# kdexd/probnmn-clevr

Hardware: AMD Instinct MI355X
Metric: CLEVR questions/sec (joint_training step) (higher is better)
Workload: dtype f32; 1 GPU; joint_training_ours.yml (NMN + seq2seq + REINFORCE), global batch 1024 = 1024 questions per GPU x 1 (BASELINE configs[3]), 14x14x1024 features, half of the batch with program supervision, fwd+bwd+[all-reduce]+clamp+Adam; global_batch=1024, per_gpu_batch=1024, parallelism=dp1

## Files before the change

include/probnmn_hip.h:

```cpp
#ifndef PROBNMN_HIP_H
#define PROBNMN_HIP_H

#include <stdint.h>

#ifdef __cplusplus
extern "C" {
#endif

#define PNMN_EINVAL (-1)
#define PNMN_ESHAPE (-2)

#define PNMN_CHANNELS 128

typedef struct pnmn_conv_item {
    const float* in;
    const float* in2;
    const float* mask;
    const float* gate;
    const float* weight;
    const float* bias;
    float*       out;
    int32_t      dilation;
    int32_t      flags;
    const float* mb_feats;
// ... 111 lines not shown
int pnmn_gather_features(const float* store, const int64_t* indices, float* dst, int n, int64_t n_store,
                         int C, int HW, void* stream);
int pnmn_copy_rows_h2d(const void* store, const int64_t* indices, void* dst, int n, int64_t n_store,
                       int64_t row_bytes, void* stream);

int pnmn_maxpool2_flatten_fwd(const float* in, float* out, int n, int H, int W, int C, void* stream);
int pnmn_maxpool2_flatten_bwd(const float* in, const float* dout, float* din, int n, int H, int W,
                              int C, void* stream);

int pnmn_answer_loss(const float* logits, const int64_t* answers, const int32_t* valid,
                     int64_t* predictions, float* loss, float* dlogits, int n, int num_answers,
                     int unknown_index, float scale, void* stream);

typedef struct {
    const float* src;
    const float* src2;
    float* dst;
    int32_t n, k, ld, kind;
} pnmn_derive_job;

int pnmn_token_prep(const int64_t* tokens, int64_t token_row_stride, int B, int T, int pad, int bos, int eos,
                    int drop_first, int64_t* out, float* fmask, int* last, void* stream);
int pnmn_length_order(const int32_t* last, int B, int T, int32_t* order, int32_t* tile_steps, void* stream);
int pnmn_trim_predictions(const int64_t* raw, int B, int T, int end, int64_t* out, void* stream);
int pnmn_mask_last_fwd(const float* hs, const float* fmask, const int* last, int B, int T, int H, float* enc,
                       float* hlast, void* stream);
int pnmn_mask_last_bwd(const float* denc, const float* dhlast, const float* fmask, const int* last, int B, int T,
                       int H, float* dhs, void* stream);
int64_t pnmn_embedding_grad_workspace_bytes(int B, int T, int V);
int pnmn_embedding_grad(const float* dy, const int64_t* tokens, int64_t token_row_stride, int B, int T, int C,
                        int V, int shift, int start, int skip, int accumulate, float* dw, void* workspace, void* stream);
int pnmn_derive_params(const pnmn_derive_job* jobs, int n_jobs, int max_quads, void* stream);

int pnmn_token_table_fwd(const float* emb, const float* weight, int64_t weight_row_stride,
                         const float* bias, int V, int K, int N, float* table, void* stream);
int pnmn_token_table_bwd(const float* dtable, const float* emb, const float* weight,
                         int64_t weight_row_stride, int V, int K, int N, int padding_idx, float* demb,
                         float* dweight, int64_t dweight_row_stride , float* dbias,
                         float* dbias2 , void* stream);

#define PNMN_TOKEN_SEGS 4
typedef struct pnmn_token_seg {
    const int64_t* src;
    const int64_t* index;
    int64_t        row_stride;
    int32_t        rows;
// ... 287 lines not shown
#define PNMN_GEMM_A_TRANSPOSED 1
#define PNMN_GEMM_B_TRANSPOSED 2
#define PNMN_GEMM_ACCUMULATE   4
typedef struct pnmn_gemm_desc {
    const float* a;
    const float* b;
    float*       c;
    const float* bias;
    int64_t      lda, ldb, ldc;
    int32_t      M, N, K;
    int32_t      flags;
    int32_t      split_k;
    int32_t      shift_t;
    const float* shift_h0;
    int64_t      ld_h0;
    float*       workspace;
    float*       colsum;
    float*       colsum2;
} pnmn_gemm_desc;
int pnmn_gemm(const pnmn_gemm_desc* descs , int n, void* stream);
int pnmn_gemm_cus(const pnmn_gemm_desc* descs , int n, int max_workgroups, void* stream);
int64_t pnmn_gemm_workspace_bytes(int M, int N, int split_k);
int pnmn_gemm_split_k(int M, int N, int K, int cus);

int pnmn_colsum(const float* x, int64_t ld, int R, int C, float* out, float* out2, int accumulate, void* workspace, void* stream);
int64_t pnmn_colsum_workspace_bytes(int R, int C);

#define PNMN_ABI_VERSION 13
int pnmn_abi_version(void);

#ifdef __cplusplus
}
#endif
#endif
```

probnmn-clevr_amd/csrc/gemm.hip:

```cpp
#include <hip/hip_runtime.h>
#include <stdint.h>

#include <type_traits>

#include "../../include/probnmn_hip.h"
#include "global_ptr.h"
#include "lds_optin.h"

namespace {

typedef float f32x16 __attribute__((ext_vector_type(16)));
using pnmn::as_global;
using pnmn::gfloat;

constexpr int TM = 128, TN = 128, TK = 32;
constexpr int OP_FLOATS = TM * TK;
using lchar = __attribute__((address_space(3))) char;
using gchar = __attribute__((address_space(1))) char;

struct Batch {
    pnmn_gemm_desc d[PNMN_GEMM_MAX];
    int first[PNMN_GEMM_MAX + 1];
    int n;
};
// ... 100 lines not shown
            const int c = (lane & 7) ^ (lane >> 4);
            base = o + ((int64_t)(row0 + 32 * wave) * ld + k0) * 4;
            v0 = (uint32_t)((lane >> 3) * ld) * 4u + 16u * c, v1 = (uint32_t)((lane >> 3) * ld) * 4u + 16u * (c ^ 4);
            piece = 32 * ld, step = 4 * TK, off = (uint32_t)wave * 32u * 128u;
        } else {
            base = o + ((int64_t)(k0 + 8 * wave) * ld + row0) * 4;
            v0 = v1 = (uint32_t)((lane >> 5) * ld) * 4u + 16u * (lane & 31);
            piece = 8 * ld, step = 4 * (int64_t)TK * ld, off = (uint32_t)wave * 8u * 512u;
        }
    }
    __device__ __forceinline__ void issue(float* tile) {
        const uint32_t dst = __builtin_amdgcn_readfirstlane((uint32_t)(uintptr_t)((lchar*)tile)) + off;
#pragma unroll
        for (int j = 0; j < 4; ++j) {
            const uint64_t src = (uint64_t)(uintptr_t)(base + j * piece);
            asm volatile("s_mov_b32 m0, %2\n\ts_nop 0\n\tglobal_load_lds_dwordx4 %0, %1"
                         :
                         : "v"(KC && (j & 1) ? v1 : v0), "s"(src), "s"(dst + 1024u * j)
                         : "memory");
        }
        base += step;
    }
};

template <bool AKC, bool BKC>
__device__ __forceinline__ void contract(const pnmn_gemm_desc& d, int m0, int n0, int kbeg, int kend, float* lds, f32x16 (&acc)[2][2],
                                         bool want_cs, float (&cs)[2]) {
    const int tid = threadIdx.x, wave = tid >> 6, lane = tid & 63, i = lane & 31, h = lane >> 5;
    const int wm = wave >> 1, wn = wave & 1;
    const gfloat* A = as_global(d.a);
    const gfloat* Bm = as_global(d.b);
    const gfloat* h0 = as_global(d.shift_h0);
    const bool avec = (d.lda & 3) == 0 && ((uintptr_t)d.a & 15) == 0;
    const bool bvec = (d.ldb & 3) == 0 && ((uintptr_t)d.b & 15) == 0 && (d.shift_t == 0 || d.shift_h0 == nullptr ||
                                                                       ((d.ld_h0 & 3) == 0 && ((uintptr_t)d.shift_h0 & 15) == 0));
    float* la = lds;
    float* lb = lds + 2 * OP_FLOATS;
    const bool adir = avec && m0 + TM <= d.M, bdir = bvec && n0 + TN <= d.N && (BKC || d.shift_t == 0);
    const int kfull = kbeg + (kend - kbeg) / TK * TK;
    const float rcp_t = d.shift_t > 0 ? 1.f / (float)d.shift_t : 0.f;
    Direct<AKC> da;
    Direct<BKC> db;
    da.start(A, d.lda, m0, kbeg, tid);
    db.start(Bm, d.ldb, n0, kbeg, tid);
    auto loop = [&](auto ad_tag, auto bd_tag, int lo, int hi) {
        constexpr bool AD = decltype(ad_tag)::value, BD = decltype(bd_tag)::value;
// ... 5 lines not shown
                load_tile<AKC>(A, d.lda, m0, k0, d.M, kend, avec, tid, ra, 0, nullptr, 0);
            if constexpr (BD)
                db.issue(lb + st * OP_FLOATS);
            else if constexpr (AD && !BKC)
                load_tile_shift(Bm, d.ldb, n0, k0, tid, rb, d.shift_t, rcp_t, h0, d.ld_h0);
            else
                load_tile<BKC>(Bm, d.ldb, n0, k0, d.N, kend, bvec, tid, rb, BKC ? 0 : d.shift_t, h0, d.ld_h0);
        };
        auto commit = [&](int st) {
            if constexpr (!AD) store_tile<AKC>(la + st * OP_FLOATS, tid, ra);
            if constexpr (!BD) store_tile<BKC>(lb + st * OP_FLOATS, tid, rb);
        };
        if (lo >= hi) return;
        fetch(lo, 0);
        commit(0);
        asm volatile("s_waitcnt vmcnt(0)" ::: "memory");
        __syncthreads();
        int cur = 0;
        for (int k0 = lo; k0 < hi; k0 += TK) {
            const bool more = k0 + TK < hi;
            if (more) fetch(k0 + TK, cur ^ 1);
            const float* ca = la + cur * OP_FLOATS;
            const float* cb = lb + cur * OP_FLOATS;
#pragma unroll
            for (int q = 0; q < 4; ++q) {
                f32x4 a[2], b[2];
#pragma unroll
                for (int t = 0; t < 2; ++t) {
                    a[t] = frag<AKC>(ca, 64 * wm + 32 * t + i, q, h);
                    b[t] = frag<BKC>(cb, 64 * wn + 32 * t + i, q, h);
                }
                if (!AKC && want_cs) {
#pragma unroll
                    for (int t = 0; t < 2; ++t) cs[t] += (a[t][0] + a[t][1]) + (a[t][2] + a[t][3]);
                }
#pragma unroll
                for (int s = 0; s < 4; ++s)
#pragma unroll
                    for (int mt = 0; mt < 2; ++mt)
#pragma unroll
                        for (int nt = 0; nt < 2; ++nt)
                            acc[mt][nt] = __builtin_amdgcn_mfma_f32_32x32x2f32(a[mt][s], b[nt][s], acc[mt][nt], 0, 0, 0);
            }
            if (more) commit(cur ^ 1);
            asm volatile("s_waitcnt vmcnt(0)" ::: "memory");
            __syncthreads();
            cur ^= 1;
        }
    };
    using yes = std::true_type;
    using no = std::false_type;
    if (adir && bdir) {
        loop(yes{}, yes{}, kbeg, kfull);
        loop(no{}, no{}, kfull, kend);
    } else if (!BKC && adir && bvec && d.shift_t > 0 && n0 + TN <= d.N && kend <= (1 << 21)) {
        if constexpr (!BKC) {
            loop(yes{}, no{}, kbeg, kfull);
            loop(no{}, no{}, kfull, kend);
        }
    } else {
        loop(no{}, no{}, kbeg, kend);
    }
}

__global__ __launch_bounds__(256) __attribute__((amdgpu_waves_per_eu(2, 2))) void gemm_kernel(const Batch batch) {
    extern __shared__ __attribute__((aligned(16))) float lds[];
    for (int unit = blockIdx.x; unit < batch.first[batch.n]; unit += gridDim.x) {
    int pi = 0;
    while (pi + 1 < batch.n && unit >= batch.first[pi + 1]) ++pi;
    const pnmn_gemm_desc d = batch.d[pi];
    const int local = unit - batch.first[pi];
    const int tiles_n = (d.N + TN - 1) / TN, tiles_m = (d.M + TM - 1) / TM;
    const int split = d.split_k > 1 ? d.split_k : 1;
    const int chunk = local % split, tile = local / split;
    const int tm = tile / tiles_n, tn = tile % tiles_n;
    const int m0 = tm * TM, n0 = tn * TN;
    const int ktiles = (d.K + TK - 1) / TK;
    const int per = ktiles / split, extra = ktiles % split;
    const int kt0 = chunk * per + (chunk < extra ? chunk : extra);
    const int kt1 = kt0 + per + (chunk < extra ? 1 : 0);
    const int kbeg = kt0 * TK, kend = kt1 * TK < d.K ? kt1 * TK : d.K;

    f32x16 acc[2][2];
#pragma unroll
    for (int mt = 0; mt < 2; ++mt)
#pragma unroll
        for (int nt = 0; nt < 2; ++nt)
#pragma unroll
            for (int r = 0; r < 16; ++r) acc[mt][nt][r] = 0.f;
    const bool akc = !(d.flags & PNMN_GEMM_A_TRANSPOSED), bkc = (d.flags & PNMN_GEMM_B_TRANSPOSED) != 0;
    const bool want_cs = d.colsum != nullptr && !akc && tn == 0 && ((threadIdx.x >> 6) & 1) == 0;
    const bool tile_cs = d.colsum != nullptr && !akc && tn == 0;
    float cs[2] = {0.f, 0.f};
    if (kbeg < kend) {
        if (akc && bkc)
            contract<true, true>(d, m0, n0, kbeg, kend, lds, acc, false, cs);
        else if (akc)
            contract<true, false>(d, m0, n0, kbeg, kend, lds, acc, false, cs);
        else if (bkc)
            contract<false, true>(d, m0, n0, kbeg, kend, lds, acc, want_cs, cs);
        else
            contract<false, false>(d, m0, n0, kbeg, kend, lds, acc, want_cs, cs);
    }

    int tid = threadIdx.x, m0e = m0, n0e = n0;
    asm volatile("" : "+v"(tid), "+s"(m0e), "+s"(n0e));
    const int wave = tid >> 6, lane = tid & 63, i = lane & 31, h = lane >> 5;
    const int wm = wave >> 1, wn = wave & 1;
    if (tile_cs) {
        if (want_cs) {
#pragma unroll
            for (int t = 0; t < 2; ++t) lds[h * TM + 64 * wm + 32 * t + i] = cs[t];
        }
        __syncthreads();
        if (tid < TM) {
            const float t = lds[tid] + lds[TM + tid];
            if (split > 1) {
// ... 149 lines not shown
    if (out2) out2[c] = total;
}

}

extern "C" int64_t pnmn_gemm_workspace_bytes(int M, int N, int split_k) {
    if (split_k <= 1) return 0;
    const int64_t tiles_m = (M + TM - 1) / TM, tiles = tiles_m * ((N + TN - 1) / TN);
    return (tiles * split_k * (TM * TN) + tiles_m * split_k * TM) * (int64_t)sizeof(float);
}

extern "C" int pnmn_gemm_split_k(int M, int N, int K, int cus) {
    const int64_t tiles = (int64_t)((M + TM - 1) / TM) * ((N + TN - 1) / TN);
    const int ktiles = (K + TK - 1) / TK;
    if (cus <= 0) cus = 256;
    int64_t want = (2 * (int64_t)cus + tiles - 1) / tiles;
    if (tiles >= cus) want = 1;
    const int most = ktiles / 4 > 0 ? ktiles / 4 : 1;
    if (want > most) want = most;
    if (want > 64) want = 64;
    return want < 1 ? 1 : (int)want;
}

extern "C" int pnmn_gemm(const pnmn_gemm_desc* descs, int n, void* stream) { return pnmn_gemm_cus(descs, n, 0, stream); }

extern "C" int pnmn_gemm_cus(const pnmn_gemm_desc* descs, int n, int max_workgroups, void* stream) {
    if (n <= 0) return 0;
    if (!descs || n > PNMN_GEMM_MAX) return PNMN_EINVAL;
    Batch b;
    int blocks = 0, live = 0;
    for (int k = 0; k < n; ++k) {
        const pnmn_gemm_desc& d = descs[k];
        if (d.M <= 0 || d.N <= 0) continue;
        if (!d.a || !d.b || !d.c || d.K < 0) return PNMN_EINVAL;
        if (d.split_k > 1 && !d.workspace) return PNMN_EINVAL;
        if (d.shift_t > 0 && (d.flags & PNMN_GEMM_B_TRANSPOSED)) return PNMN_ESHAPE;
        if (d.colsum && !(d.flags & PNMN_GEMM_A_TRANSPOSED)) return PNMN_ESHAPE;
        b.d[live] = d;
        b.first[live] = blocks;
        const int tiles = ((d.M + TM - 1) / TM) * ((d.N + TN - 1) / TN);
        blocks += tiles * (d.split_k > 1 ? d.split_k : 1);
        ++live;
    }
    if (!live) return 0;
    b.first[live] = blocks;
    b.n = live;
    constexpr size_t lds = (size_t)4 * OP_FLOATS * sizeof(float);
    static std::atomic<uint64_t> cfg{0};
    if (const int e = pnmn::opt_in_lds(reinterpret_cast<const void*>(gemm_kernel), lds, cfg)) return e;
    const int grid = (max_workgroups > 0 && max_workgroups < blocks) ? max_workgroups : blocks;
    hipLaunchKernelGGL(gemm_kernel, dim3(grid), dim3(256), lds, static_cast<hipStream_t>(stream), b);
    Batch r;
    int rblocks = 0, rlive = 0;
    for (int k = 0; k < live; ++k) {
        if (b.d[k].split_k <= 1) continue;
        r.d[rlive] = b.d[k];
        r.first[rlive] = rblocks;
        rblocks += 4 * ((b.d[k].M + TM - 1) / TM) * ((b.d[k].N + TN - 1) / TN);
        ++rlive;
    }
    if (rlive) {
        r.first[rlive] = rblocks;
        r.n = rlive;
        hipLaunchKernelGGL(gemm_reduce_kernel, dim3(rblocks), dim3(256), 0, static_cast<hipStream_t>(stream), r);
    }
    return (int)hipGetLastError();
}

extern "C" int64_t pnmn_colsum_workspace_bytes(int R, int C) {
    (void)R;
    return (int64_t)128 * C * sizeof(float) + (int64_t)((C + 255) / 256) * sizeof(int);
}

extern "C" int pnmn_colsum(const float* x, int64_t ld, int R, int C, float* out, float* out2, int accumulate, void* workspace,
                           void* stream) {
    if (C <= 0) return 0;
    if (!out || !workspace || (R > 0 && !x)) return PNMN_EINVAL;
    int slices = (R + 63) / 64;
    if (slices > 128) slices = 128;
    if (slices < 1) slices = 1;
    float* partial = static_cast<float*>(workspace);
    int* counter = reinterpret_cast<int*>(partial + (size_t)128 * C);
    const int vec = (ld & 3) == 0 && ((uintptr_t)x & 15) == 0;
    hipLaunchKernelGGL(colsum_kernel, dim3((C + 255) / 256, slices), dim3(256), 0, static_cast<hipStream_t>(stream), x, ld, R, C,
                       partial, counter, out, out2, accumulate, vec);
    return (int)hipGetLastError();
}
```

probnmn-clevr_amd/csrc/seqglue.hip:

```cpp
#include <hip/hip_runtime.h>
#include <stdint.h>
#include <stdlib.h>

#include "../../include/probnmn_hip.h"

namespace {

__global__ __launch_bounds__(256) void token_prep_kernel(const int64_t* __restrict__ tokens, int64_t tstride, int B, int T,
                                                         int pad, int bos, int eos, int drop_first,
                                                         int64_t* __restrict__ out, float* __restrict__ fmask,
                                                         int* __restrict__ last) {
    const int b = blockIdx.x * 4 + (threadIdx.x >> 6);
    const int lane = threadIdx.x & 63;
    if (b >= B) return;
    const int64_t* row = tokens + (size_t)b * tstride;
    int n = 0;
    for (int t = lane; t < T; t += 64) n += row[t] != pad;
#pragma unroll
    for (int o = 32; o > 0; o >>= 1) n += __shfl_xor(n, o);
    const int W = T + 2 - drop_first;
    int valid = 0;
    for (int j = lane; j < W; j += 64) {
        const int f = j + drop_first;
        int64_t v = (f == 0) ? bos : (f <= T ? row[f - 1] : 0);
// ... 85 lines not shown
        carry += __shfl(incl, 63);
    }
    __syncthreads();
    for (int b0 = 0; b0 < B; b0 += 64) {
        const int b = b0 + lane;
        const int s = b < B ? min(max(last[b] + 1, 1), T) : 0;
        int before = 0, after = 0;
        for (int j = 0; j < 64; ++j) {
            const int sj = __shfl(s, j);
            before += (sj == s && j < lane);
            after += (sj == s && j > lane);
        }
        const int pos = s ? first[s] + before : 0;
        __syncthreads();
        if (s) {
            order[pos] = b;
            if ((pos & 15) == 0) tile_steps[pos >> 4] = s;
            if (after == 0) first[s] = pos + 1;
        }
        __syncthreads();
    }
}

__global__ __launch_bounds__(256) void mask_last_bwd_kernel(const float* __restrict__ denc, const float* __restrict__ dhlast,
                                                            const float* __restrict__ fmask, const int* __restrict__ last,
                                                            int T, int H, float* __restrict__ dhs) {
    const int b = blockIdx.x;
    int l = last[b];
    if (l < 0) l += T;
    const int h4 = H >> 2;
    const float4* src = denc ? reinterpret_cast<const float4*>(denc + (size_t)b * T * H) : nullptr;
    float4* dst = reinterpret_cast<float4*>(dhs + (size_t)b * T * H);
    for (int i = blockIdx.y * 256 + threadIdx.x; i < T * h4; i += gridDim.y * 256) {
        const int t = i / h4;
        const float m = fmask[(size_t)b * T + t];
        float4 v = src ? src[i] : float4{0.f, 0.f, 0.f, 0.f};
        if (dhlast && t == l) {
            const float4 d = reinterpret_cast<const float4*>(dhlast + (size_t)b * H)[i - t * h4];
            v.x += d.x, v.y += d.y, v.z += d.z, v.w += d.w;
        }
        v.x *= m, v.y *= m, v.z *= m, v.w *= m;
        dst[i] = v;
    }
}

constexpr int EG_CHUNK = 64;
// ... 212 lines not shown
            const float sum = (lds[r * 17 + c] + lds[(16 + r) * 17 + c]) + (lds[(32 + r) * 17 + c] + lds[(48 + r) * 17 + c]);
            demb[(size_t)v * K + 16 * kt + c] = v == padding_idx ? 0.f : sum;
        }
    }
}

}

extern "C" int pnmn_token_prep(const int64_t* tokens, int64_t token_row_stride, int B, int T, int pad, int bos, int eos,
                               int drop_first, int64_t* out, float* fmask, int* last, void* stream) {
    if (B <= 0) return 0;
    if (!tokens || !out || T < 0) return PNMN_EINVAL;
    hipLaunchKernelGGL(token_prep_kernel, dim3((B + 3) / 4), dim3(256), 0, static_cast<hipStream_t>(stream), tokens,
                       token_row_stride, B, T, pad, bos, eos, drop_first, out, fmask, last);
    return (int)hipGetLastError();
}

extern "C" int pnmn_length_order(const int32_t* last, int B, int T, int32_t* order, int32_t* tile_steps, void* stream) {
    if (B <= 0) return 0;
    if (!last || !order || !tile_steps || T <= 0) return PNMN_EINVAL;
    if (T > LO_MAX_T) return PNMN_ESHAPE;
    hipLaunchKernelGGL(length_order_kernel, dim3(1), dim3(64), (size_t)(T + 1) * sizeof(int), static_cast<hipStream_t>(stream),
                       last, B, T, order, tile_steps);
    return (int)hipGetLastError();
}

extern "C" int pnmn_token_rows(const pnmn_token_seg* segs, int n_segs, int64_t* dst, int W, int64_t pad, void* stream) {
    if (n_segs <= 0 || W <= 0) return 0;
    if (!segs || !dst || n_segs > PNMN_TOKEN_SEGS) return PNMN_EINVAL;
    TokenSegs t;
    int total = 0;
    for (int k = 0; k < n_segs; ++k) {
        if (segs[k].rows < 0 || (segs[k].rows > 0 && !segs[k].src) || segs[k].width < 0) return PNMN_EINVAL;
        t.s[k] = segs[k];
        total += segs[k].rows;
    }
    t.n = n_segs;
    if (total == 0) return 0;
    hipLaunchKernelGGL(token_rows_kernel, dim3((total + 3) / 4), dim3(256), 0, static_cast<hipStream_t>(stream), t, dst, W, pad,
                       total);
    return (int)hipGetLastError();
}

extern "C" int pnmn_trim_predictions(const int64_t* raw, int B, int T, int end, int64_t* out, void* stream) {
    if (B <= 0 || T <= 0) return 0;
    if (!raw || !out) return PNMN_EINVAL;
// ... 131 lines not shown
```

probnmn-clevr_amd/probnmn/runtime/seq_plan.py:

```python
import os
from dataclasses import dataclass
from typing import Dict, List, NamedTuple, Optional

import numpy as np
import torch

from probnmn import _hip


SPLIT_SLOTS = int(os.environ.get("PNMN_PLAN_SPLIT_SLOTS", "512"))
SPLIT_MIN_KTILES = int(os.environ.get("PNMN_PLAN_SPLIT_MIN", "8"))
USE_STACK = True
STACK_FWD_ENCODERS = int(os.environ.get("PNMN_PLAN_FWD_ENC", "2"))
STACK_PG_ENCODER = int(os.environ.get("PNMN_PLAN_PG_ENC", "1"))
STACK_BWD_ENCODERS = int(os.environ.get("PNMN_PLAN_BWD_ENC", "0"))
LENGTH_ORDER_ABOVE_ROWS = 256
DECODER_BUFFERS = (("hs", 256), ("cs", 256), ("cx", 256), ("act", 1024), ("dhs", 256), ("dg", 1024), ("dctx", 256))


class PlanUnsupported(Exception):
    """The models / shapes are outside what the plan is built for: the trainer keeps the eager passes."""


class _Calls(list):
    def add(self, name: str, *args) -> None:
        self.append((getattr(_hip.lib(), name), args, name))

    def add_fn(self, name: str, fn) -> None:
        self.append((fn, (), name))

    def run(self) -> None:
        for fn, args, name in self:
            rc = fn(*args)
            if rc:
                _hip.check(rc, name)


def _supported(model) -> bool:
    lstm, cell = model._encoder._module, model._decoder_cell
# ... 115 lines not shown
    p: float = 0.0


class Seq2SeqPlan:

    def __init__(self, pg, qr, prior, dev: torch.device, n: int, m: int, tq: int, tp: int):
        if not (_supported(pg) and _supported(qr)) or n <= 0 or m <= 0:
            raise PlanUnsupported("model shapes")
        pl = prior._encoder._module
        if pl.hidden_size != 256 or pl.num_layers != 2 or pl.input_size != 256:
            raise PlanUnsupported("prior shapes")
        if pl.training and _dropout_p(pl) > 0:
            raise PlanUnsupported("prior in training mode with dropout")
        self.dev, self.n, self.m, self.tq, self.tp = dev, n, m, tq, tp
        self.stream = _hip.stream_ptr(dev)
        self.pg, self.qr, self.prior = _Model(pg, dev), _Model(qr, dev), prior
        self.drop_p = (_dropout_p(pg._encoder._module), _dropout_p(qr._encoder._module))
        self.B, self.D = n + m, pg._max_decoding_steps
        if _hip.decoder_workspace_bytes([n, m], False) <= 0 or _hip.decoder_workspace_bytes([self.B], False) <= 0 \
                or int(_hip.lib().pnmn_lstm_seq_workspace_bytes(self.B, 0)) <= 0:
            raise PlanUnsupported("batch does not fit the multi-CU recurrent kernels in one launch")
        self._bufs: Dict[str, torch.Tensor] = {}
        self._keep: List = []
        self.anchor = torch.zeros((), device=dev, requires_grad=True)
        self.fwd_pg_enc, self.fwd_pg, self.fwd_pg_finish, self.fwd_qr, self.fwd_prior = (_Calls() for _ in range(5))
        self.bwd_a, self.bwd_b = _Calls(), _Calls()
        self._build()

    def buf(self, name: str, *shape, dtype=torch.float32, zero: bool = False) -> torch.Tensor:
        if name in self._bufs:
            raise KeyError(name)
        t = (torch.zeros if zero else torch.empty)(*shape, dtype=dtype, device=self.dev)
        self._bufs[name] = t
        return t

    def bytes_buf(self, name: str, nbytes: int, zero: bool = False) -> torch.Tensor:
        return self.buf(name, max(int(nbytes), 16), dtype=torch.uint8, zero=zero)

    def __getitem__(self, name: str) -> torch.Tensor:
        return self._bufs[name]

    def _gemm(self, calls: _Calls, name: str, descs) -> None:
        lib = _hip.lib()
        for lo in range(0, len(descs), _hip.GEMM_MAX):
            part = descs[lo:lo + _hip.GEMM_MAX]
            rec = np.zeros(len(part), _hip.GEMM_DESC)
# ... 7 lines not shown
                units = fixed_units + sum(tiles[i] * sp for i, sp in zip(auto, splits))
                longest = max([-(-ktiles[i] // sp) for i, sp in zip(auto, splits)] + [ktiles[i] for i in range(len(part)) if i not in auto] + [1])
                rounds = units // SPLIT_SLOTS + (0.6 if units % SPLIT_SLOTS else 0.0)
                cost = rounds * longest + 4.0 * sum(tiles[i] * sp for i, sp in zip(auto, splits) if sp > 1) / SPLIT_SLOTS
                if best is None or cost < best:
                    chunk_len, best = cand, cost
            for i, d in enumerate(part):
                r = rec[i]
                r["a"], r["b"], r["c"] = d["a"], d["b"], d["c"]
                r["lda"], r["ldb"], r["ldc"] = d["lda"], d["ldb"], d["ldc"]
                r["M"], r["N"], r["K"] = d["M"], d["N"], d["K"]
                r["flags"] = (_hip.GEMM_A_T if d.get("ta") else 0) | (_hip.GEMM_B_T if d.get("tb") else 0) | (_hip.GEMM_ACC if d.get("acc") else 0)
                r["bias"] = d.get("bias", 0)
                split = d.get("split", 1)
                if split == "auto":
                    split = max(1, min(-(-ktiles[i] // chunk_len), 64))
                r["split_k"] = split
                if split > 1:
                    ws = self.bytes_buf("%s.ws%d" % (name, lo + i), lib.pnmn_gemm_workspace_bytes(d["M"], d["N"], split), zero=True)
                    r["workspace"] = ws.data_ptr()
                r["shift_t"], r["shift_h0"], r["ld_h0"] = d.get("shift_t", 0), d.get("h0", 0), d.get("ld_h0", 0)
                r["colsum"], r["colsum2"] = d.get("colsum", 0), d.get("colsum2", 0)
            self._keep.append(rec)
            calls.add("pnmn_gemm_cus", rec.ctypes.data, len(rec), 0, self.stream)

    def _table_forward(self, calls: _Calls, t: _TokenTable) -> None:
        calls.add("pnmn_token_table_fwd", t.emb.data_ptr(), t.w_ih.data_ptr() + 4 * t.col0, t.w_ih.stride(0), t.bias.data_ptr(),
                  t.emb.size(0), 256, 1024, t.table.data_ptr(), self.stream)

    def _table_backward(self, calls: _Calls, t: _TokenTable, mm: _Model, start: int, uses) -> None:
        V, g = t.emb.size(0), mm.grad
        dtable = self.buf(t.tag + ".dtable", V, 1024)
        for k, (ws_name, dg, tokens, shift) in enumerate(uses):
            rows, T = dg.shape[:2]
            ews = self.bytes_buf(ws_name, _hip.lib().pnmn_embedding_grad_workspace_bytes(rows, T, V))
            calls.add("pnmn_embedding_grad", dg.data_ptr(), tokens.data_ptr(), tokens.stride(0), rows, T, 1024, V, shift, start, -1,
                      1 if k else 0, dtable.data_ptr(), ews.data_ptr(), self.stream)
        ld = t.w_ih.stride(0)
        calls.add("pnmn_token_table_bwd", dtable.data_ptr(), t.emb.data_ptr(), t.w_ih.data_ptr() + 4 * t.col0, ld, V, 256, 1024, t.pad_idx,
                  g(t.emb).data_ptr(), g(t.w_ih).data_ptr() + 4 * t.col0, ld if ld != 256 else 0, g(t.b_ih).data_ptr(),
                  g(t.b_hh).data_ptr(), self.stream)

    def _encoder_prepare(self, calls: _Calls, ep: _EncoderPass) -> Dict:
        model, derived = (ep.mm.model, ep.mm.derived) if ep.mm is not None else (self.prior, self.prior._derived())
        tag, rows, lstm, emb, f = ep.tag, ep.rows, model._encoder._module, ep.embedding.weight, self.buf
        T, V = ep.width + 2 - int(ep.drop_first), emb.size(0)
        e = dict(tag=tag, mm=ep.mm, derived=derived, lstm=lstm, T=T, rows=rows, want_last=ep.want_last,
# ... 119 lines not shown
            e["dhs2"], e["dg2"], e["dg1"] = f(tag + ".dhs2", rows, T, 256), f(tag + ".dg2", rows, T, 1024), f(tag + ".dg1", rows, T, 1024)
            calls.add("pnmn_mask_last_bwd", e["denc"].data_ptr(), e["dh"].data_ptr(), e["fmask"].data_ptr(), e["last"].data_ptr(), rows, T, 256,
                      e["dhs2"].data_ptr(), st)
        for e in self._stack_launches(calls, name, encs, True):
            d, lstm, tag, rows, T = e["derived"], e["lstm"], e["tag"], e["rows"], e["T"]
            dhs1 = f(tag + ".dhs1", rows, T, 256)
            ws = self.bytes_buf(tag + ".lstm_bws", lib.pnmn_lstm_seq_workspace_bytes(rows, 1))
            bwd, ordered = ("pnmn_lstm_seq_bwd_ordered", (e["order"].data_ptr(), e["tile_steps"].data_ptr())) if "order" in e else ("pnmn_lstm_seq_bwd", ())
            calls.add(bwd, e["dhs2"].data_ptr(), e["act2"].data_ptr(), e["cs2"].data_ptr(), d["l1.hhT"].data_ptr(),
                      e["dg2"].data_ptr(), rows, T, 256, *ordered, ws.data_ptr(), st)
            self._gemm(calls, tag + ".dx", [dict(a=e["dg2"].data_ptr(), b=lstm.weight_ih_l1.data_ptr(), c=dhs1.data_ptr(), M=rows * T, N=256,
                                                 K=1024, lda=1024, ldb=256, ldc=256, split="auto")])
            if e["p"] > 0:
                self._dropout_call(calls, e, dhs1, dhs1)
            calls.add(bwd, dhs1.data_ptr(), e["act1"].data_ptr(), e["cs1"].data_ptr(), d["l0.hhT"].data_ptr(),
                      e["dg1"].data_ptr(), rows, T, 256, *ordered, ws.data_ptr(), st)

    def _encoders_param_grads(self, calls: _Calls, deferred: List, encs: List[Dict]) -> None:
        for e in encs:
            mm, lstm, rows, T = e["mm"], e["lstm"], e["rows"], e["T"]
            dg1, dg2, g = e["dg1"], e["dg2"], mm.grad
            self._table_backward(calls, e["tab"], mm, 0, [(e["tag"] + ".emb_ws", dg1, e["src"], 0)])
            K = rows * T
            deferred += [
                dict(a=dg2.data_ptr(), b=e["hs2"].data_ptr(), c=g(lstm.weight_hh_l1).data_ptr(), M=1024, N=256, K=K, lda=1024, ldb=256,
                     ldc=256, ta=1, split="auto", shift_t=T, colsum=g(lstm.bias_ih_l1).data_ptr(), colsum2=g(lstm.bias_hh_l1).data_ptr()),
                dict(a=dg2.data_ptr(), b=(e["hsd"] if e["p"] > 0 else e["hs1"]).data_ptr(), c=g(lstm.weight_ih_l1).data_ptr(), M=1024,
                     N=256, K=K, lda=1024, ldb=256, ldc=256, ta=1, split="auto"),
                dict(a=dg1.data_ptr(), b=e["hs1"].data_ptr(), c=g(lstm.weight_hh_l0).data_ptr(), M=1024, N=256, K=K, lda=1024, ldb=256,
                     ldc=256, ta=1, split="auto", shift_t=T),
            ]

    def _decoder_set(self, tag: str, mm: _Model, enc: Dict, passes) -> _DecoderSet:
        f, S, V = self.buf, enc["T"], mm.proj.weight.size(0)
        R = sum(rows * T for _, _, rows, T, _, _ in passes)
        table = _TokenTable(tag + ".d", mm.emb_tgt, mm.cell.weight_ih, 256, mm.cell.bias_ih, mm.cell.bias_hh, mm.derived["d.b"], -1,
                            f(tag + ".d.table", V, 1024))
        dec = _DecoderSet(tag, mm, enc, table, {k: f("%s.d.%s" % (tag, k), R, w) for k, w in DECODER_BUFFERS},
                          f(tag + ".logits", R, V), f(tag + ".dlogits", R, V), [])
        row0 = enc_row0 = 0
        for ptag, suffix, rows, T, tokens, trimmed in passes:
            v = {k: dec.flat[k][row0:row0 + rows * T].view(rows, T, w) for k, w in DECODER_BUFFERS}
            for k in ("probs", "dscore", "weights"):
                v[k] = f("%s.%s" % (ptag, k), rows, T, S)
            target = tokens.data_ptr() + (0 if trimmed is not None else 8)
            loss = _Loss(dec.logits[row0:], T * V, target, tokens.stride(0), target if trimmed is None else trimmed.data_ptr(),
                         tokens.stride(0), mm.model._pad_index, f("%s.loss%s" % (tag, suffix), rows), f("%s.lse%s" % (tag, suffix), rows, T),
                         rows, T, V, 1e-13 if trimmed is None else 1e-12)
            dec.passes.append(_DecoderPass(ptag, rows, T, S, row0, enc_row0, tokens, int(trimmed is not None), trimmed, v, loss))
            row0, enc_row0 = row0 + rows * T, enc_row0 + rows
        return dec

    def _decoder_fwd_job(self, j, dec: _DecoderSet, p: _DecoderPass) -> None:
# ... 112 lines not shown
        bj = np.zeros(len(passes), _hip.DECODER_BWD_JOB)
        for j, (dec, p) in zip(bj, passes):
            e, r0 = dec.enc, p.enc_row0
            j["dhs"], j["act"], j["cs"], j["hs"], j["probs"] = (p.v[k].data_ptr() for k in ("dhs", "act", "cs", "hs", "probs"))
            j["enc"], j["mask"], j["h0"] = e["enc"][r0:].data_ptr(), e["fmask"][r0:].data_ptr(), e["h"][r0:].data_ptr()
            j["w_c_t"], j["w_hh_t"] = dec.mm.derived["d.cT"].data_ptr(), dec.mm.derived["d.hhT"].data_ptr()
            j["dgates"], j["dctx"], j["dscore"], j["weights"] = (p.v[k].data_ptr() for k in ("dg", "dctx", "dscore", "weights"))
            j["dh0"] = e["dh"][r0:].data_ptr()
            j["B"], j["T"], j["S"] = p.rows, p.T, p.S
        self._keep.append(bj)
        gws = self.bytes_buf("group_ws", _hip.decoder_workspace_bytes([p.rows for _, p in passes], True))
        c.add("pnmn_attn_lstm_bwd_group", bj.ctypes.data, len(bj), 256, gws.data_ptr(), st)
        for dec, p in passes:
            c.add("pnmn_attn_denc", p.v["weights"].data_ptr(), p.v["dscore"].data_ptr(), p.v["dctx"].data_ptr(), p.v["hs"].data_ptr(),
                  dec.enc["h"][p.enc_row0:].data_ptr(), dec.enc["denc"][p.enc_row0:].data_ptr(), p.rows, p.T, p.S, 256, st)
        self._encoders_bwd(self.bwd_b, "enc", [dec.enc for dec in decs])

    def _parameter_gradients(self, decs: List[_DecoderSet]) -> None:
        c, deferred = self.bwd_b, []
        for dec in decs:
            mm, flat, (R, V), g, cell = dec.mm, dec.flat, dec.logits.shape, dec.mm.grad, dec.mm.cell
            self._table_backward(c, dec.table, mm, mm.model._start_index,
                                 [("%s.d.emb_ws%d" % (dec.tag, k), p.v["dg"], p.tokens, p.shift) for k, p in enumerate(dec.passes)])
            deferred.append(dict(a=dec.dlogits.data_ptr(), b=flat["hs"].data_ptr(), c=g(mm.proj.weight).data_ptr(), M=V, N=256, K=R, lda=V,
                                 ldb=256, ldc=256, ta=1, split="auto", colsum=g(mm.proj.bias).data_ptr()))
            deferred.append(dict(a=flat["dg"].data_ptr(), b=flat["cx"].data_ptr(), c=g(cell.weight_ih).data_ptr(), M=1024, N=256, K=R, lda=1024,
                                 ldb=256, ldc=512, ta=1, split="auto"))
            for k, p in enumerate(dec.passes):
                deferred.append(dict(a=p.v["dg"].data_ptr(), b=p.v["hs"].data_ptr(), c=g(cell.weight_hh).data_ptr(), M=1024, N=256,
                                     K=p.rows * p.T, lda=1024, ldb=256, ldc=256, ta=1, split="auto", shift_t=p.T,
                                     h0=dec.enc["h"][p.enc_row0:].data_ptr(), ld_h0=256, acc=1 if k else 0))
        self._encoders_param_grads(c, deferred, [dec.enc for dec in decs])
        self._gemm(c, "wgrad", [d for d in deferred if not d.get("acc")])
        self._gemm(c, "wgrad2", [d for d in deferred if d.get("acc")])

    def _sig(self):
        return tuple(t.data_ptr() for model in (self.pg.model, self.qr.model, self.prior) for t in model._derived().values())

    def still_valid(self) -> bool:
        if _hip.stream_ptr(self.dev) != self.stream:
            return False
        for mm in (self.pg, self.qr):
            if tuple(p.data_ptr() for p in mm.params) != mm.signature:
                return False
        if tuple(p.data_ptr() for p in self.prior.parameters()) != self.prior_sig:
            return False
        if (_dropout_p(self.pg.lstm), _dropout_p(self.qr.lstm)) != self.drop_p:
            return False
        if self.prior.training and _dropout_p(self.prior._encoder._module) > 0:
            return False
        return self._sig() == self._derived_sig

    def run_encoder(self, question: torch.Tensor, program: torch.Tensor, nosup_d: torch.Tensor, sup_d: torch.Tensor) -> None:
        lib, st = _hip.lib(), self.stream
        if question.dtype != torch.long or program.dtype != torch.long or question.stride(1) != 1 or program.stride(1) != 1:
# ... 62 lines not shown
```

Baseline: 37750 questions/s.

## Skip padded timesteps in weight-gradient GEMMs via compacted valid-row lists

Adds a kernel that builds, on the device, a compact list of (row, shifted-row) pairs for the non-padded timesteps of each encoder and decoder pass. A list-driven GEMM variant then gathers only those rows along K for the LSTM and projection weight-gradient GEMMs, so padded positions are no longer contracted. This costs an extra small launch, indirect row loads, and a K that is only known on the device, which can leave split-K chunks unbalanced or empty.

```diff
diff --git a/include/probnmn_hip.h b/include/probnmn_hip.h
--- a/include/probnmn_hip.h
+++ b/include/probnmn_hip.h
@@ -157,6 +157,10 @@
 int pnmn_token_prep(const int64_t* tokens, int64_t token_row_stride, int B, int T, int pad, int bos, int eos,
                     int drop_first, int64_t* out, float* fmask, int* last, void* stream);
 int pnmn_length_order(const int32_t* last, int B, int T, int32_t* order, int32_t* tile_steps, void* stream);
+int pnmn_valid_rows(const int32_t* const* last , const int64_t* const* mask_tokens ,
+                    const int64_t* mask_stride , const int32_t* pad ,
+                    const int32_t* rows , const int32_t* T , int32_t* const* list ,
+                    int32_t* const* count , int n, void* stream);
 int pnmn_trim_predictions(const int64_t* raw, int B, int T, int end, int64_t* out, void* stream);
 int pnmn_mask_last_fwd(const float* hs, const float* fmask, const int* last, int B, int T, int H, float* enc,
                        float* hlast, void* stream);
@@ -490,6 +494,8 @@
 int pnmn_gemm_cus(const pnmn_gemm_desc* descs , int n, int max_workgroups, void* stream);
 int64_t pnmn_gemm_workspace_bytes(int M, int N, int split_k);
 int pnmn_gemm_split_k(int M, int N, int K, int cus);
+int pnmn_gemm_rows(const pnmn_gemm_desc* descs , int n, const int32_t* const* rows ,
+                   const int32_t* const* count , int max_workgroups, void* stream);
 
 int pnmn_colsum(const float* x, int64_t ld, int R, int C, float* out, float* out2, int accumulate, void* workspace, void* stream);
 int64_t pnmn_colsum_workspace_bytes(int R, int C);
diff --git a/probnmn-clevr_amd/csrc/gemm.hip b/probnmn-clevr_amd/csrc/gemm.hip
--- a/probnmn-clevr_amd/csrc/gemm.hip
+++ b/probnmn-clevr_amd/csrc/gemm.hip
@@ -146,6 +146,31 @@
         base += step;
     }
 };
+
+template <bool AKC, bool BKC>
+__device__ __forceinline__ void mac_tile(const float* ca, const float* cb, int wm, int wn, int i, int h, f32x16 (&acc)[2][2], bool want_cs,
+                                         float (&cs)[2]) {
+#pragma unroll
+    for (int q = 0; q < 4; ++q) {
+        f32x4 a[2], b[2];
+#pragma unroll
+        for (int t = 0; t < 2; ++t) {
+            a[t] = frag<AKC>(ca, 64 * wm + 32 * t + i, q, h);
+            b[t] = frag<BKC>(cb, 64 * wn + 32 * t + i, q, h);
+        }
+        if (!AKC && want_cs) {
+#pragma unroll
+            for (int t = 0; t < 2; ++t) cs[t] += (a[t][0] + a[t][1]) + (a[t][2] + a[t][3]);
+        }
+#pragma unroll
+        for (int s = 0; s < 4; ++s)
+#pragma unroll
+            for (int mt = 0; mt < 2; ++mt)
+#pragma unroll
+                for (int nt = 0; nt < 2; ++nt)
+                    acc[mt][nt] = __builtin_amdgcn_mfma_f32_32x32x2f32(a[mt][s], b[nt][s], acc[mt][nt], 0, 0, 0);
+    }
+}
 
 template <bool AKC, bool BKC>
 __device__ __forceinline__ void contract(const pnmn_gemm_desc& d, int m0, int n0, int kbeg, int kend, float* lds, f32x16 (&acc)[2][2],
@@ -197,26 +222,7 @@
             if (more) fetch(k0 + TK, cur ^ 1);
             const float* ca = la + cur * OP_FLOATS;
             const float* cb = lb + cur * OP_FLOATS;
-#pragma unroll
-            for (int q = 0; q < 4; ++q) {
-                f32x4 a[2], b[2];
-#pragma unroll
-                for (int t = 0; t < 2; ++t) {
-                    a[t] = frag<AKC>(ca, 64 * wm + 32 * t + i, q, h);
-                    b[t] = frag<BKC>(cb, 64 * wn + 32 * t + i, q, h);
-                }
-                if (!AKC && want_cs) {
-#pragma unroll
-                    for (int t = 0; t < 2; ++t) cs[t] += (a[t][0] + a[t][1]) + (a[t][2] + a[t][3]);
-                }
-#pragma unroll
-                for (int s = 0; s < 4; ++s)
-#pragma unroll
-                    for (int mt = 0; mt < 2; ++mt)
-#pragma unroll
-                        for (int nt = 0; nt < 2; ++nt)
-                            acc[mt][nt] = __builtin_amdgcn_mfma_f32_32x32x2f32(a[mt][s], b[nt][s], acc[mt][nt], 0, 0, 0);
-            }
+            mac_tile<AKC, BKC>(ca, cb, wm, wn, i, h, acc, want_cs, cs);
             if (more) commit(cur ^ 1);
             asm volatile("s_waitcnt vmcnt(0)" ::: "memory");
             __syncthreads();
@@ -238,7 +244,136 @@
     }
 }
 
-__global__ __launch_bounds__(256) __attribute__((amdgpu_waves_per_eu(2, 2))) void gemm_kernel(const Batch batch) {
+using gint2 = __attribute__((address_space(1))) int2;
+
+__device__ __forceinline__ void load_rows(const gint2* list, int k0, int kend, int tid, int2 (&e)[4]) {
+#pragma unroll
+    for (int j = 0; j < 4; ++j) {
+        const int k = k0 + (tid >> 5) + 8 * j;
+        const gint2* q = list + (k < kend ? k : kend - 1);
+        e[j].x = q->x, e[j].y = q->y;
+    }
+}
+
+__device__ __forceinline__ void load_tile_rows(const gfloat* base, int64_t ld, int col0, int k0, int cols, int kend, bool vec, int tid,
+                                               const int2 (&e)[4], f32x4 (&r)[4], bool shifted, const gfloat* h0, int64_t ld_h0) {
+#pragma unroll
+    for (int j = 0; j < 4; ++j) {
+        const int k = k0 + (tid >> 5) + 8 * j, col = col0 + 4 * (tid & 31);
+        f32x4 v = f32x4{0.f, 0.f, 0.f, 0.f};
+        if (k < kend && col < cols) {
+            const int row = shifted ? e[j].y : e[j].x;
+            const bool first = row < 0;
+            const gfloat* src = first ? (h0 ? h0 + (int64_t)(~row) * ld_h0 + col : base + col) : base + (int64_t)row * ld + col;
+            if (vec && col + 3 < cols) {
+                v = pnmn::load4(src);
+            } else {
+#pragma unroll
+                for (int c = 0; c < 4; ++c)
+                    if (col + c < cols) v[c] = src[c];
+            }
+            if (first && !h0) v = f32x4{0.f, 0.f, 0.f, 0.f};
+        }
+        r[j] = v;
+    }
+}
+
+struct DirectRows {
+    const gchar* origin;
+    int64_t ld;
+    uint32_t lane, off;
+
+    __device__ __forceinline__ void start(const gfloat* base, int64_t ld_floats, int col0, int tid) {
+        origin = (const gchar*)(base + col0), ld = 4 * ld_floats;
+        lane = 16u * (tid & 31), off = (uint32_t)__builtin_amdgcn_readfirstlane(tid >> 6) * 1024u;
+    }
+    __device__ __forceinline__ void issue(float* tile, const int2 (&e)[4]) {
+        const uint32_t dst = __builtin_amdgcn_readfirstlane((uint32_t)(uintptr_t)((lchar*)tile)) + off;
+#pragma unroll
+        for (int j = 0; j < 4; ++j) {
+            const gchar* src = origin + (int64_t)e[j].x * ld + lane;
+            asm volatile("s_mov_b32 m0, %1\n\ts_nop 0\n\tglobal_load_lds_dwordx4 %0, off" : : "v"(src), "s"(dst + 4096u * j) : "memory");
+        }
+    }
+};
+
+__device__ __forceinline__ void contract_rows(const pnmn_gemm_desc& d, const gint2* list, int m0, int n0, int kbeg, int kend, float* lds,
+                                              f32x16 (&acc)[2][2], bool want_cs, float (&cs)[2]) {
+    const int tid = threadIdx.x, wave = tid >> 6, lane = tid & 63, i = lane & 31, h = lane >> 5;
+    const int wm = wave >> 1, wn = wave & 1;
+    const gfloat* A = as_global(d.a);
+    const gfloat* Bm = as_global(d.b);
+    const gfloat* h0 = as_global(d.shift_h0);
+    const bool shifted = d.shift_t > 0;
+    const bool avec = (d.lda & 3) == 0 && ((uintptr_t)d.a & 15) == 0;
+    const bool bvec = (d.ldb & 3) == 0 && ((uintptr_t)d.b & 15) == 0 &&
+                      (!shifted || d.shift_h0 == nullptr || ((d.ld_h0 & 3) == 0 && ((uintptr_t)d.shift_h0 & 15) == 0));
+    float* la = lds;
+    float* lb = lds + 2 * OP_FLOATS;
+    const bool adir = avec && m0 + TM <= d.M, bdir = bvec && n0 + TN <= d.N && !shifted;
+    const int kfull = kbeg + (kend - kbeg) / TK * TK;
+    DirectRows da, db;
+    da.start(A, d.lda, m0, tid);
+    db.start(Bm, d.ldb, n0, tid);
+    auto loop = [&](auto ad_tag, auto bd_tag, int lo, int hi) {
+        constexpr bool AD = decltype(ad_tag)::value, BD = decltype(bd_tag)::value;
+        f32x4 ra[4], rb[4];
+        int2 e[4];
+        auto fetch = [&](int k0, int st) {
+            if constexpr (AD)
+                da.issue(la + st * OP_FLOATS, e);
+            else
+                load_tile_rows(A, d.lda, m0, k0, d.M, kend, avec, tid, e, ra, false, nullptr, 0);
+            if constexpr (BD)
+                db.issue(lb + st * OP_FLOATS, e);
+            else
+                load_tile_rows(Bm, d.ldb, n0, k0, d.N, kend, bvec, tid, e, rb, shifted, h0, d.ld_h0);
+        };
+        auto commit = [&](int st) {
+            if constexpr (!AD) store_tile<false>(la + st * OP_FLOATS, tid, ra);
+            if constexpr (!BD) store_tile<false>(lb + st * OP_FLOATS, tid, rb);
+        };
+        if (lo >= hi) return;
+        load_rows(list, lo, kend, tid, e);
+        fetch(lo, 0);
+        load_rows(list, lo + TK, kend, tid, e);
+        commit(0);
+        asm volatile("s_waitcnt vmcnt(0)" ::: "memory");
+        __syncthreads();
+        int cur = 0;
+        for (int k0 = lo; k0 < hi; k0 += TK) {
+            const bool more = k0 + TK < hi;
+            if (more) {
+                fetch(k0 + TK, cur ^ 1);
+                load_rows(list, k0 + 2 * TK, kend, tid, e);
+            }
+            mac_tile<false, false>(la + cur * OP_FLOATS, lb + cur * OP_FLOATS, wm, wn, i, h, acc, want_cs, cs);
+            if (more) commit(cur ^ 1);
+            asm volatile("s_waitcnt vmcnt(0)" ::: "memory");
+            __syncthreads();
+            cur ^= 1;
+        }
+    };
+    using yes = std::true_type;
+    using no = std::false_type;
+    if (adir && bdir) {
+        loop(yes{}, yes{}, kbeg, kfull);
+        loop(no{}, no{}, kfull, kend);
+    } else if (adir) {
+        loop(yes{}, no{}, kbeg, kfull);
+        loop(no{}, no{}, kfull, kend);
+    } else {
+        loop(no{}, no{}, kbeg, kend);
+    }
+}
+
+struct Lists {
+    const int2* rows[PNMN_GEMM_MAX];
+    const int32_t* count[PNMN_GEMM_MAX];
+};
+
+template <bool LIST>
+__global__ __launch_bounds__(256) __attribute__((amdgpu_waves_per_eu(2, 2))) void gemm_kernel(const Batch batch, const Lists lists) {
     extern __shared__ __attribute__((aligned(16))) float lds[];
     for (int unit = blockIdx.x; unit < batch.first[batch.n]; unit += gridDim.x) {
     int pi = 0;
@@ -250,11 +385,20 @@
     const int chunk = local % split, tile = local / split;
     const int tm = tile / tiles_n, tn = tile % tiles_n;
     const int m0 = tm * TM, n0 = tn * TN;
-    const int ktiles = (d.K + TK - 1) / TK;
+    int K = d.K;
+    const gint2* list = nullptr;
+    if constexpr (LIST) {
+        list = (const gint2*)lists.rows[pi];
+        if (list) {
+            const int count = __builtin_amdgcn_readfirstlane(*(const __attribute__((address_space(1))) int32_t*)lists.count[pi]);
+            K = count < 0 ? 0 : (count < d.K ? count : d.K);
+        }
+    }
+    const int ktiles = (K + TK - 1) / TK;
     const int per = ktiles / split, extra = ktiles % split;
     const int kt0 = chunk * per + (chunk < extra ? chunk : extra);
     const int kt1 = kt0 + per + (chunk < extra ? 1 : 0);
-    const int kbeg = kt0 * TK, kend = kt1 * TK < d.K ? kt1 * TK : d.K;
+    const int kbeg = kt0 * TK, kend = kt1 * TK < K ? kt1 * TK : K;
 
     f32x16 acc[2][2];
 #pragma unroll
@@ -267,7 +411,9 @@
     const bool want_cs = d.colsum != nullptr && !akc && tn == 0 && ((threadIdx.x >> 6) & 1) == 0;
     const bool tile_cs = d.colsum != nullptr && !akc && tn == 0;
     float cs[2] = {0.f, 0.f};
-    if (kbeg < kend) {
+    if (LIST && list) {
+        if (kbeg < kend) contract_rows(d, list, m0, n0, kbeg, kend, lds, acc, want_cs, cs);
+    } else if (kbeg < kend) {
         if (akc && bkc)
             contract<true, true>(d, m0, n0, kbeg, kend, lds, acc, false, cs);
         else if (akc)
@@ -463,12 +609,14 @@
     return want < 1 ? 1 : (int)want;
 }
 
-extern "C" int pnmn_gemm(const pnmn_gemm_desc* descs, int n, void* stream) { return pnmn_gemm_cus(descs, n, 0, stream); }
-
-extern "C" int pnmn_gemm_cus(const pnmn_gemm_desc* descs, int n, int max_workgroups, void* stream) {
+namespace {
+int launch(const pnmn_gemm_desc* descs, int n, const int32_t* const* rows, const int32_t* const* count, int max_workgroups,
+           void* stream) {
     if (n <= 0) return 0;
     if (!descs || n > PNMN_GEMM_MAX) return PNMN_EINVAL;
     Batch b;
+    Lists l = {};
+    bool listed = false;
     int blocks = 0, live = 0;
     for (int k = 0; k < n; ++k) {
         const pnmn_gemm_desc& d = descs[k];
@@ -477,6 +625,13 @@
         if (d.split_k > 1 && !d.workspace) return PNMN_EINVAL;
         if (d.shift_t > 0 && (d.flags & PNMN_GEMM_B_TRANSPOSED)) return PNMN_ESHAPE;
         if (d.colsum && !(d.flags & PNMN_GEMM_A_TRANSPOSED)) return PNMN_ESHAPE;
+        l.rows[live] = nullptr, l.count[live] = nullptr;
+        if (rows && rows[k]) {
+            if ((d.flags & (PNMN_GEMM_A_TRANSPOSED | PNMN_GEMM_B_TRANSPOSED)) != PNMN_GEMM_A_TRANSPOSED) return PNMN_ESHAPE;
+            if (!count || !count[k]) return PNMN_EINVAL;
+            l.rows[live] = reinterpret_cast<const int2*>(rows[k]), l.count[live] = count[k];
+            listed = true;
+        }
         b.d[live] = d;
         b.first[live] = blocks;
         const int tiles = ((d.M + TM - 1) / TM) * ((d.N + TN - 1) / TN);
@@ -487,10 +642,15 @@
     b.first[live] = blocks;
     b.n = live;
     constexpr size_t lds = (size_t)4 * OP_FLOATS * sizeof(float);
-    static std::atomic<uint64_t> cfg{0};
-    if (const int e = pnmn::opt_in_lds(reinterpret_cast<const void*>(gemm_kernel), lds, cfg)) return e;
+    static std::atomic<uint64_t> cfg{0}, cfg_rows{0};
     const int grid = (max_workgroups > 0 && max_workgroups < blocks) ? max_workgroups : blocks;
-    hipLaunchKernelGGL(gemm_kernel, dim3(grid), dim3(256), lds, static_cast<hipStream_t>(stream), b);
+    if (listed) {
+        if (const int e = pnmn::opt_in_lds(reinterpret_cast<const void*>(gemm_kernel<true>), lds, cfg_rows)) return e;
+        hipLaunchKernelGGL(gemm_kernel<true>, dim3(grid), dim3(256), lds, static_cast<hipStream_t>(stream), b, l);
+    } else {
+        if (const int e = pnmn::opt_in_lds(reinterpret_cast<const void*>(gemm_kernel<false>), lds, cfg)) return e;
+        hipLaunchKernelGGL(gemm_kernel<false>, dim3(grid), dim3(256), lds, static_cast<hipStream_t>(stream), b, l);
+    }
     Batch r;
     int rblocks = 0, rlive = 0;
     for (int k = 0; k < live; ++k) {
@@ -506,6 +666,18 @@
         hipLaunchKernelGGL(gemm_reduce_kernel, dim3(rblocks), dim3(256), 0, static_cast<hipStream_t>(stream), r);
     }
     return (int)hipGetLastError();
+}
+}
+
+extern "C" int pnmn_gemm(const pnmn_gemm_desc* descs, int n, void* stream) { return launch(descs, n, nullptr, nullptr, 0, stream); }
+
+extern "C" int pnmn_gemm_cus(const pnmn_gemm_desc* descs, int n, int max_workgroups, void* stream) {
+    return launch(descs, n, nullptr, nullptr, max_workgroups, stream);
+}
+
+extern "C" int pnmn_gemm_rows(const pnmn_gemm_desc* descs, int n, const int32_t* const* rows, const int32_t* const* count,
+                              int max_workgroups, void* stream) {
+    return launch(descs, n, rows, count, max_workgroups, stream);
 }
 
 extern "C" int64_t pnmn_colsum_workspace_bytes(int R, int C) {
diff --git a/probnmn-clevr_amd/csrc/seqglue.hip b/probnmn-clevr_amd/csrc/seqglue.hip
--- a/probnmn-clevr_amd/csrc/seqglue.hip
+++ b/probnmn-clevr_amd/csrc/seqglue.hip
@@ -131,6 +131,71 @@
     }
 }
 
+constexpr int VR_SEGS = 8;
+struct ValidSegs {
+    const int32_t* last[VR_SEGS];
+    const int64_t* mask[VR_SEGS];
+    int64_t mask_stride[VR_SEGS];
+    int2* list[VR_SEGS];
+    int32_t* count[VR_SEGS];
+    int32_t pad[VR_SEGS], rows[VR_SEGS], T[VR_SEGS];
+    int32_t first[VR_SEGS + 1];
+};
+__global__ __launch_bounds__(1024) void valid_rows_kernel(const ValidSegs s) {
+    __shared__ int wsum[16], steps_of[1024], first_of[1024];
+    const int tid = threadIdx.x, wave = tid >> 6, lane = tid & 63;
+    const int seg0 = s.first[blockIdx.x], seg1 = s.first[blockIdx.x + 1];
+    int2* list = s.list[seg0];
+    int entries = 0, row_base = 0, seq_base = 0;
+    for (int g = seg0; g < seg1; ++g) {
+        const int rows = s.rows[g], T = s.T[g], pad = s.pad[g];
+        const int32_t* last = s.last[g];
+        for (int b0 = 0; b0 < rows; b0 += 1024) {
+            const int b = b0 + tid;
+            int steps = 0;
+            if (b < rows) {
+                if (last) {
+                    steps = min(max(last[b] + 1, 1), T);
+                } else {
+                    const int64_t* m = s.mask[g] + (int64_t)b * s.mask_stride[g];
+                    for (int t0 = 0; t0 < T; t0 += 8) {
+                        int64_t v[8];
+#pragma unroll
+                        for (int u = 0; u < 8; ++u) v[u] = m[min(t0 + u, T - 1)];
+#pragma unroll
+                        for (int u = 0; u < 8; ++u)
+                            if (t0 + u < T && v[u] != pad) steps = t0 + u + 1;
+                    }
+                }
+            }
+            int incl = steps;
+#pragma unroll
+            for (int o = 1; o < 64; o <<= 1) {
+                const int v = __shfl_up(incl, o);
+                if (lane >= o) incl += v;
+            }
+            if (lane == 63) wsum[wave] = incl;
+            __syncthreads();
+            int before = 0, total = 0;
+            for (int w = 0; w < 16; ++w) {
+                before += w < wave ? wsum[w] : 0;
+                total += wsum[w];
+            }
+            steps_of[tid] = steps, first_of[tid] = entries + before + incl - steps;
+            __syncthreads();
+            const int nb = min(1024, rows - b0);
+            for (int r = wave; r < nb; r += 16) {
+                const int n = steps_of[r], o = first_of[r], row0 = row_base + (b0 + r) * T;
+                for (int t = lane; t < n; t += 64) list[o + t] = int2{row0 + t, t ? row0 + t - 1 : ~(seq_base + b0 + r)};
+            }
+            entries += total;
+            __syncthreads();
+        }
+        row_base += rows * T, seq_base += rows;
+    }
+    if (tid == 0) *s.count[seg0] = entries;
+}
+
 __global__ __launch_bounds__(256) void mask_last_bwd_kernel(const float* __restrict__ denc, const float* __restrict__ dhlast,
                                                             const float* __restrict__ fmask, const int* __restrict__ last,
                                                             int T, int H, float* __restrict__ dhs) {
@@ -389,6 +454,32 @@
     if (T > LO_MAX_T) return PNMN_ESHAPE;
     hipLaunchKernelGGL(length_order_kernel, dim3(1), dim3(64), (size_t)(T + 1) * sizeof(int), static_cast<hipStream_t>(stream),
                        last, B, T, order, tile_steps);
+    return (int)hipGetLastError();
+}
+
+extern "C" int pnmn_valid_rows(const int32_t* const* last, const int64_t* const* mask_tokens, const int64_t* mask_stride,
+                               const int32_t* pad, const int32_t* rows, const int32_t* T, int32_t* const* list, int32_t* const* count,
+                               int n, void* stream) {
+    if (n <= 0) return 0;
+    if (n > VR_SEGS || !last || !mask_tokens || !mask_stride || !pad || !rows || !T || !list || !count) return PNMN_EINVAL;
+    ValidSegs s;
+    int lists = 0;
+    int64_t total = 0;
+    for (int k = 0; k < n; ++k) {
+        if (rows[k] < 0 || T[k] <= 0 || !list[k] || (rows[k] > 0 && !last[k] && !mask_tokens[k])) return PNMN_EINVAL;
+        const bool appended = k > 0 && list[k] == list[k - 1];
+        if (!appended) {
+            if (!count[k]) return PNMN_EINVAL;
+            s.first[lists++] = k, total = 0;
+        }
+        total += (int64_t)rows[k] * T[k];
+        if (total >= (1LL << 31)) return PNMN_ESHAPE;
+        s.last[k] = last[k], s.mask[k] = mask_tokens[k], s.mask_stride[k] = mask_stride[k];
+        s.list[k] = reinterpret_cast<int2*>(list[k]), s.count[k] = count[k];
+        s.pad[k] = pad[k], s.rows[k] = rows[k], s.T[k] = T[k];
+    }
+    s.first[lists] = n;
+    hipLaunchKernelGGL(valid_rows_kernel, dim3(lists), dim3(1024), 0, static_cast<hipStream_t>(stream), s);
     return (int)hipGetLastError();
 }
 
diff --git a/probnmn-clevr_amd/probnmn/runtime/seq_plan.py b/probnmn-clevr_amd/probnmn/runtime/seq_plan.py
--- a/probnmn-clevr_amd/probnmn/runtime/seq_plan.py
+++ b/probnmn-clevr_amd/probnmn/runtime/seq_plan.py
@@ -15,6 +15,7 @@
 STACK_PG_ENCODER = int(os.environ.get("PNMN_PLAN_PG_ENC", "1"))
 STACK_BWD_ENCODERS = int(os.environ.get("PNMN_PLAN_BWD_ENC", "0"))
 LENGTH_ORDER_ABOVE_ROWS = 256
+VALID_PAIRS_ABOVE_ROWS = LENGTH_ORDER_ABOVE_ROWS
 DECODER_BUFFERS = (("hs", 256), ("cs", 256), ("cx", 256), ("act", 1024), ("dhs", 256), ("dg", 1024), ("dctx", 256))
 
 
@@ -176,6 +177,9 @@
             raise PlanUnsupported("batch does not fit the multi-CU recurrent kernels in one launch")
         self._bufs: Dict[str, torch.Tensor] = {}
         self._keep: List = []
+        self._keep_args: List[np.ndarray] = []
+        self._valid_lists: List = []
+        self.valid_pairs = os.environ.get("PNMN_GEMM_VALID_PAIRS", "1") != "0"
         self.anchor = torch.zeros((), device=dev, requires_grad=True)
         self.fwd_pg_enc, self.fwd_pg, self.fwd_pg_finish, self.fwd_qr, self.fwd_prior = (_Calls() for _ in range(5))
         self.bwd_a, self.bwd_b = _Calls(), _Calls()
@@ -229,7 +233,36 @@
                 r["shift_t"], r["shift_h0"], r["ld_h0"] = d.get("shift_t", 0), d.get("h0", 0), d.get("ld_h0", 0)
                 r["colsum"], r["colsum2"] = d.get("colsum", 0), d.get("colsum2", 0)
             self._keep.append(rec)
-            calls.add("pnmn_gemm_cus", rec.ctypes.data, len(rec), 0, self.stream)
+            if any(d.get("valid") for d in part):
+                lists = np.array([d.get("valid", (0, 0)) for d in part], np.uint64).T.copy()
+                self._keep_args.append(lists)
+                calls.add("pnmn_gemm_rows", rec.ctypes.data, len(rec), lists[0].ctypes.data, lists[1].ctypes.data, 0, self.stream)
+            else:
+                calls.add("pnmn_gemm_cus", rec.ctypes.data, len(rec), 0, self.stream)
+
+    def _valid_list(self, name: str, segments) -> tuple:
+        rows = self.buf(name + ".rows", sum(r * T for _, _, _, _, r, T in segments), 2, dtype=torch.int32)
+        count = self.buf(name + ".count", 1, dtype=torch.int32, zero=True)
+        self._valid_lists.append((rows.data_ptr(), count.data_ptr(), segments))
+        return rows.data_ptr(), count.data_ptr()
+
+    def _valid_list_calls(self, calls: _Calls) -> None:
+        group: List = []
+
+        def flush():
+            if group:
+                arg = np.array(group, np.int64).T.copy()
+                pad, rows, T = (arg[k].astype(np.int32) for k in (3, 4, 5))
+                self._keep_args += [arg, pad, rows, T]
+                calls.add("pnmn_valid_rows", arg[0].ctypes.data, arg[1].ctypes.data, arg[2].ctypes.data, pad.ctypes.data, rows.ctypes.data,
+                          T.ctypes.data, arg[6].ctypes.data, arg[7].ctypes.data, len(group), self.stream)
+                del group[:]
+        for lst, count, segments in self._valid_lists:
+            if len(group) + len(segments) > 8:
+                flush()
+            group += [seg + (lst, count) for seg in segments]
+        flush()
+        self._valid_lists = []
 
     def _table_forward(self, calls: _Calls, t: _TokenTable) -> None:
         calls.add("pnmn_token_table_fwd", t.emb.data_ptr(), t.w_ih.data_ptr() + 4 * t.col0, t.w_ih.stride(0), t.bias.data_ptr(),
@@ -395,13 +428,15 @@
             dg1, dg2, g = e["dg1"], e["dg2"], mm.grad
             self._table_backward(calls, e["tab"], mm, 0, [(e["tag"] + ".emb_ws", dg1, e["src"], 0)])
             K = rows * T
+            valid = dict(valid=self._valid_list(e["tag"] + ".valid", [(e["last"].data_ptr(), 0, 0, 0, rows, T)])) \
+                if self.valid_pairs and rows > VALID_PAIRS_ABOVE_ROWS else {}
             deferred += [
                 dict(a=dg2.data_ptr(), b=e["hs2"].data_ptr(), c=g(lstm.weight_hh_l1).data_ptr(), M=1024, N=256, K=K, lda=1024, ldb=256,
-                     ldc=256, ta=1, split="auto", shift_t=T, colsum=g(lstm.bias_ih_l1).data_ptr(), colsum2=g(lstm.bias_hh_l1).data_ptr()),
+                     ldc=256, ta=1, split="auto", shift_t=T, colsum=g(lstm.bias_ih_l1).data_ptr(), colsum2=g(lstm.bias_hh_l1).data_ptr(), **valid),
                 dict(a=dg2.data_ptr(), b=(e["hsd"] if e["p"] > 0 else e["hs1"]).data_ptr(), c=g(lstm.weight_ih_l1).data_ptr(), M=1024,
-                     N=256, K=K, lda=1024, ldb=256, ldc=256, ta=1, split="auto"),
+                     N=256, K=K, lda=1024, ldb=256, ldc=256, ta=1, split="auto", **valid),
                 dict(a=dg1.data_ptr(), b=e["hs1"].data_ptr(), c=g(lstm.weight_hh_l0).data_ptr(), M=1024, N=256, K=K, lda=1024, ldb=256,
-                     ldc=256, ta=1, split="auto", shift_t=T),
+                     ldc=256, ta=1, split="auto", shift_t=T, **valid),
             ]
 
     def _decoder_set(self, tag: str, mm: _Model, enc: Dict, passes) -> _DecoderSet:
@@ -560,15 +595,21 @@
             mm, flat, (R, V), g, cell = dec.mm, dec.flat, dec.logits.shape, dec.mm.grad, dec.mm.cell
             self._table_backward(c, dec.table, mm, mm.model._start_index,
                                  [("%s.d.emb_ws%d" % (dec.tag, k), p.v["dg"], p.tokens, p.shift) for k, p in enumerate(dec.passes)])
+            segs = [(0, p.loss.mask, p.loss.mask_stride, p.loss.pad, p.rows, p.T) for p in dec.passes]
+            listed = self.valid_pairs and sum(p.rows for p in dec.passes) > VALID_PAIRS_ABOVE_ROWS
+            whole = dict(valid=self._valid_list(dec.tag + ".d.valid", segs)) if listed else {}
+            own = [whole if len(segs) == 1 else dict(valid=self._valid_list(p.tag + ".valid", [seg])) if listed else {}
+                   for p, seg in zip(dec.passes, segs)]
             deferred.append(dict(a=dec.dlogits.data_ptr(), b=flat["hs"].data_ptr(), c=g(mm.proj.weight).data_ptr(), M=V, N=256, K=R, lda=V,
-                                 ldb=256, ldc=256, ta=1, split="auto", colsum=g(mm.proj.bias).data_ptr()))
+                                 ldb=256, ldc=256, ta=1, split="auto", colsum=g(mm.proj.bias).data_ptr(), **whole))
             deferred.append(dict(a=flat["dg"].data_ptr(), b=flat["cx"].data_ptr(), c=g(cell.weight_ih).data_ptr(), M=1024, N=256, K=R, lda=1024,
-                                 ldb=256, ldc=512, ta=1, split="auto"))
+                                 ldb=256, ldc=512, ta=1, split="auto", **whole))
             for k, p in enumerate(dec.passes):
                 deferred.append(dict(a=p.v["dg"].data_ptr(), b=p.v["hs"].data_ptr(), c=g(cell.weight_hh).data_ptr(), M=1024, N=256,
                                      K=p.rows * p.T, lda=1024, ldb=256, ldc=256, ta=1, split="auto", shift_t=p.T,
-                                     h0=dec.enc["h"][p.enc_row0:].data_ptr(), ld_h0=256, acc=1 if k else 0))
+                                     h0=dec.enc["h"][p.enc_row0:].data_ptr(), ld_h0=256, acc=1 if k else 0, **own[k]))
         self._encoders_param_grads(c, deferred, [dec.enc for dec in decs])
+        self._valid_list_calls(c)
         self._gemm(c, "wgrad", [d for d in deferred if not d.get("acc")])
         self._gemm(c, "wgrad2", [d for d in deferred if d.get("acc")])
 
```

New measurement: 38660 questions/s, median of 6. +2.4%, better.
